# diver-j/melgan-multi

Measured on NVIDIA H100. Metric: generator_fwd_audio_frames_per_sec, higher is better.
Workload: dtype f32 in/out; products as 3 split-bf16 wgmma passes with fp32 accumulation (fp32-equivalent, ~1e-5)

## Files before the change

melgan_multi_b200/csrc/mg_common.cuh:

```cuda
#pragma once
#include <cuda_runtime.h>
#include <stdarg.h>
#include <stdint.h>
#include <stdio.h>

#include "../../include/melgan_b200.h"
#include "mg_layout.h"

namespace mg {

constexpr int kNumSMs = 132;

char *error_buffer();
int set_error(int code, const char *fmt, ...);

#define MG_CUDA_TRY(expr)                                                                     \
    do {                                                                                      \
        cudaError_t err__ = (expr);                                                           \
        if (err__ != cudaSuccess)                                                             \
            return ::mg::set_error(MG_ERR_CUDA, "%s failed: %s (%s:%d)", #expr,               \
                                   cudaGetErrorString(err__), __FILE__, __LINE__);            \
    } while (0)

__device__ __forceinline__ float lrelu(float x) { return fmaxf(x, x * kSlope); }

__device__ __forceinline__ void cp_async16(void *smem_dst, const void *gmem_src) {
    uint32_t d = (uint32_t)__cvta_generic_to_shared(smem_dst);
    asm volatile("cp.async.cg.shared.global [%0], [%1], 16;\n" ::"r"(d), "l"(gmem_src));
}
__device__ __forceinline__ void cp_async_commit() { asm volatile("cp.async.commit_group;\n" ::); }
template <int N>
__device__ __forceinline__ void cp_async_wait() {
    asm volatile("cp.async.wait_group %0;\n" ::"n"(N));
}

bool pdl_enabled();
template <class... KArgs, class... Args>
inline cudaError_t launch_ex(void (*kernel)(KArgs...), dim3 grid, dim3 block, size_t smem, cudaStream_t s, bool pdl, Args... args) {
    cudaLaunchConfig_t cfg{};
    cfg.gridDim = grid;
    cfg.blockDim = block;
    cfg.dynamicSmemBytes = smem;
    cfg.stream = s;
    cudaLaunchAttribute attr[1];
    int n = 0;
    if (pdl && pdl_enabled()) {
        attr[n].id = cudaLaunchAttributeProgrammaticStreamSerialization;
        attr[n].val.programmaticStreamSerializationAllowed = 1;
        ++n;
    }
    cfg.attrs = attr;
    cfg.numAttrs = n;
    return cudaLaunchKernelEx(&cfg, kernel, static_cast<KArgs>(args)...);
}

int launch_pack(const float *const *v, const float *const *g, const float *const *bias, float *packed,
                cudaStream_t s);
int launch_generator_simt(const float *packed, const float *mel, float *audio, int B, int T, float *ws,
                          cudaStream_t s, cudaEvent_t *ev = nullptr);
int generator_simt_num_launches();
int generator_tc_num_launches();
int generator_tc_fused_up();
int generator_tc_tail();
void generator_tc_set_tail(int mask);
const char *generator_tc_kernel_name(int i);
const char *generator_tc_kernel_config(int i, int T);
const char *resblock_config_name(int stage, int L);
int generator_tc_slices(int B, int T);
int launch_generator_tc(const float *packed, const float *mel, float *audio, int B, int T, float *ws, int *status,
                        cudaStream_t s, cudaEvent_t *ev = nullptr, const float *mel_host = nullptr, float *audio_host = nullptr);
int launch_gen_pre_tc(const float *mel, float *y, const float *packed, int B, int T, int *status, cudaStream_t s);
int launch_disc_post1_tc(const float *x, float *y, const uint8_t *wtc, const float *bias, int Bt, int L, int *status,
                         cudaStream_t s);
int launch_disc_post1_dgrad_tc(const float *dz, float *dx, const uint8_t *wtcT, const float *zero_bias, int Bt, int L, int *status,
                               cudaStream_t s);
int launch_disc_post1_wgrad_tc(const float *x, const float *dz, float *dw, float *db, int Bt, int L, int *status, cudaStream_t s);
size_t disc_scale_backward_workspace_bytes(int Bt, int L0);
int launch_disc_scale_backward(const void *blob, const float *x0, const float *const *fmap, const float *const *gfmap, float *gx0,
                               float *const *dw, float *const *db, int *reached, void *workspace, size_t workspace_bytes, int Bt,
                               int L0, int *status, cudaStream_t st);
size_t edge_bwd_workspace_bytes(int l, int Bt, int L);
// ... 34 lines not shown
```

melgan_multi_b200/csrc/mg_conv_tc.cu:

```cuda
#include "mg_common.cuh"
#include "mg_tc.cuh"

namespace mg {
using namespace tc;

template <int CIN_, int COUT_, int NTAP_, int KCA_, bool LRELU_OUT_, int N_>
struct ConvCfg {
    static constexpr int CIN = CIN_, COUT = COUT_, NTAP = NTAP_, PAD = NTAP_ / 2, KCA = KCA_;
    static constexpr bool LRELU_OUT = LRELU_OUT_;
    static constexpr int N = N_;
    static constexpr int NCG = COUT / N;
    static constexpr int ROWS = 128;
    static constexpr int AROWS = ROWS + 2 * PAD + 2;
    static constexpr int APITCH = AROWS * 16;
    static constexpr int ASLOT = 2 * (KCA / 8) * APITCH;
    static constexpr int BSLOT = 2 * 2 * N * 16;
    static constexpr int NSA = (CIN == KCA) ? 1 : 2, NSB = (N_ == 128) ? 8 : 4;
    static constexpr int NCONV = 128, NMW = 2;
    static constexpr int NT = NCONV + 128 * NMW + 32;
    static constexpr int SMEM_BYTES = NSA * ASLOT + NSB * BSLOT + (2 * NSA + 2 * NSB) * 8;
    static_assert(CIN % KCA == 0 && KCA % 16 == 0 && COUT % N == 0, "shape");
    static_assert(SMEM_BYTES + 1024 <= 227 * 1024, "shared memory budget");
};

// ... 135 lines not shown
        for (int ca = 0; ca < NCH; ca += 2) {
#pragma unroll
            for (int half = 0; half < 2; ++half) {
                const int cc = ca + half;
                if (cc < NCH) {
                    float *cur = half ? fb : fa, *nxt = half ? fa : fb;
                    if (cc + 1 < NCH) {
#pragma unroll
                        for (int j = 0; j < KCA; ++j) nxt[j] = inr0 ? __ldg(xrow + (size_t)((cc + 1) * KCA + j) * L) : 0.f;
                    }
                    if (ok && !mbar_wait(&emptyA[sa], pha ^ 1)) { ok = false; if (lane == 0) atomicExch(status, 24); }
                    uint8_t *slot = aring + sa * ASLOT;
                    store_row(slot, tid, cur);
                    tail_rows(slot, cc);
                    fence_proxy_async();
                    mbar_arrive(&fullA[sa]);
                    if (++sa == NSA) { sa = 0; pha ^= 1; }
                }
            }
        }
    }
}

template <class Cfg>
static int launch_conv_rows(const float *x, float *y, const uint8_t *wtc, const float *bias, int B, int L, int *status,
                            cudaStream_t s) {
    static bool configured = false;
    if (!configured) {
        MG_CUDA_TRY(cudaFuncSetAttribute(conv_rows_tc_kernel<Cfg>, cudaFuncAttributeMaxDynamicSharedMemorySize, Cfg::SMEM_BYTES));
        configured = true;
    }
    const long long vrows = (long long)B * (L + Cfg::PAD);
    const unsigned tiles = (unsigned)((vrows + Cfg::ROWS - 1) / Cfg::ROWS);
    MG_CUDA_TRY(launch_ex(conv_rows_tc_kernel<Cfg>, dim3(tiles, Cfg::NCG), dim3(Cfg::NT), Cfg::SMEM_BYTES, s, true, x, y, wtc, bias,
                          L, B, status));
    return MG_OK;
}

using PreCfg = ConvCfg<80, 512, 7, 80, false, kPreNG>;
using Post1Cfg = ConvCfg<1024, 1024, 5, 32, true, kPost1NG>;
using Post1DgradCfg = ConvCfg<1024, 1024, 5, 32, false, kPost1NG>;

int launch_gen_pre_tc(const float *mel, float *y, const float *packed, int B, int T, int *status, cudaStream_t s) {
    const uint8_t *wtc = reinterpret_cast<const uint8_t *>(packed) + tc_region_start() + tc_pre_offset();
    return launch_conv_rows<PreCfg>(mel, y, wtc, packed + bias_offset(0), B, T, status, s);
}

int launch_disc_post1_tc(const float *x, float *y, const uint8_t *wtc, const float *bias, int Bt, int L, int *status,
                         cudaStream_t s) {
    return launch_conv_rows<Post1Cfg>(x, y, wtc, bias, Bt, L, status, s);
}

int launch_disc_post1_dgrad_tc(const float *dz, float *dx, const uint8_t *wtcT, const float *zero_bias, int Bt, int L, int *status,
                               cudaStream_t s) {
    return launch_conv_rows<Post1DgradCfg>(dz, dx, wtcT, zero_bias, Bt, L, status, s);
}

}
```

melgan_multi_b200/csrc/mg_res_tc.cu:

```cuda
#include <stdlib.h>
#include <string.h>

#include "mg_common.cuh"
#include "mg_tc.cuh"

namespace mg {
using namespace tc;

template <int C_, int NRB_, int RPW_, int NCP_, int NSTAGE_, bool POST_ = false, bool UPF_ = false, int UPT_ = 0>
struct RbCfg {
    static constexpr int C = C_, NRB = NRB_, RPW = RPW_, NCP = NCP_, NSTAGE = NSTAGE_, UPT = UPT_;
    static constexpr bool POST = POST_;
    static constexpr bool UPF = UPF_;
    static constexpr int P = 64 * NRB;
    static constexpr int NWG = NRB / RPW * NCP;
    static constexpr int NCONS = 128 * NWG;
    static constexpr int NT = NCONS + 32;
    static constexpr int NCW = C / NCP;
    static constexpr int SLACK = 16;
    static constexpr int HALO = 16 + (POST ? 3 : 0);
    static constexpr int HL = HALO + (UPT_ ? 1 : 0);
    static constexpr int PVALID = P - HALO - HL;
    static constexpr int ROWS = P + 2 * SLACK;
    static constexpr int XPITCH = ROWS * 16;
    static constexpr int KP = C / 8;
    static constexpr int XBYTES = KP * XPITCH;
    static constexpr int KC = tc_kc(C);
    static constexpr int CHUNK = tc_chunk_bytes(C);
    static constexpr int HALF = CHUNK / 2;
    static constexpr int NCHUNK = tc_chunks_per_conv(C);
    static constexpr int KSL = C / KC;
    static constexpr int TNG = UPT == 8 ? 32 : C / 2, TN = (UPT ? UPT : 1) * TNG, TNCG = (C / 2) / TNG;
    static constexpr int TSLOT = UPT == 8 ? 16384 : 128 * UPT * TNG, TNSLOT = UPT ? TNCG * (C / 16) * (UPT == 8 ? 2 : 1) : 0;
    static_assert(UPT == 0 || ((UPT == 2 || UPT == 8) && TN == C && TSLOT <= CHUNK && !POST_ && !UPF_), "tail ConvT shape");
    static_assert(UPT != 8 || NCW == 128, "stride-8 tail: each column part stores four phases of a channel as one float4");
    static constexpr int UROWS = P / 2 + 2, UPITCH = UROWS * 16, NPB = NRB / 2, UKSL = 2 * C / KC, NUPCH = UPF ? 4 * UKSL : 0;
    static constexpr int SPITCH = P + 4;
    static_assert(!UPF || (NCP == 1 && NPB <= NWG && 2 * KP * UPITCH <= XBYTES && C * SPITCH * 4 <= 2 * XBYTES),
                  "fused ConvT must fit the X region");
    static_assert(!POST || (C == 32 && NCP == 1), "conv_post fusion is for the 32-channel stage");
    static constexpr int SMEM_BYTES = 2 * XBYTES + NSTAGE * CHUNK + 2 * C * 4 + 2 * NSTAGE * 8;
    static_assert(SMEM_BYTES + 1024 <= 227 * 1024, "shared memory budget");
    static_assert(XPITCH / 16 < 16384, "LBO field");
    static_assert(NRB % RPW == 0 && C % NCP == 0 && NCW % 32 == 0, "warpgroup split");
};

template <int RPW, int R>
__device__ __forceinline__ void acc_fence2(float (&a)[RPW][R]) {
#pragma unroll
    for (int r = 0; r < RPW; ++r) acc_fence<R>(a[r]);
}

template <class Cfg>
__global__ void __launch_bounds__(Cfg::NT, 1)
resblock_tc_kernel(const float *__restrict__ x, float *__restrict__ y, const float *__restrict__ packed, int stage, int L, int nB,
                   int *__restrict__ status, long long *__restrict__ trace) {
    constexpr int C = Cfg::C, P = Cfg::P, SLACK = Cfg::SLACK, HALO = Cfg::HALO, HL = Cfg::HL, PVS = Cfg::PVALID;
    constexpr int XPITCH = Cfg::XPITCH, XBYTES = Cfg::XBYTES, KC = Cfg::KC, CHUNK = Cfg::CHUNK, NSTAGE = Cfg::NSTAGE;
    constexpr int NCONS = Cfg::NCONS, NCP = Cfg::NCP, NCW = Cfg::NCW, RPW = Cfg::RPW, KSL = Cfg::KSL, NA = NCW / 2;
    extern __shared__ __align__(1024) uint8_t smem[];
    uint8_t *Xh = smem, *Xl = smem + XBYTES, *ring = smem + 2 * XBYTES;
    float *pend = reinterpret_cast<float *>(ring + NSTAGE * CHUNK);
    float *b1s = pend + C;
    uint64_t *full = reinterpret_cast<uint64_t *>(b1s + C);
    uint64_t *empty = full + NSTAGE;

    const int tid = threadIdx.x, warp = tid >> 5, lane = tid & 31;
    const int b = blockIdx.y, stile = blockIdx.x;
    const int o = stile == 0 ? 0 : (P - HALO) + (stile - 1) * PVS - HL;
    const int p_lo = stile == 0 ? 0 : HL, p_hi = (o + P >= L) ? P : P - HALO;
    const bool interior = (o >= 0 && o + P <= L);
    const int l0 = 5 + 6 * stage;
    const uint8_t *tc_base = reinterpret_cast<const uint8_t *>(packed) + tc_region_start();

    if (tid == 0) {
        for (int s = 0; s < NSTAGE; ++s) {
            mbar_init(&full[s], 1);
            mbar_init(&empty[s], Cfg::NWG);
        }
        fence_mbar_init();
    }
    for (int i = Cfg::UPF ? 1 << 30 : tid; i < 2 * Cfg::KP * 2 * SLACK; i += Cfg::NT) {
        const int r = i % (2 * SLACK), kp = (i / (2 * SLACK)) % Cfg::KP, hl = i / (2 * SLACK * Cfg::KP);
        const int row = r < SLACK ? r : P + r;
        *reinterpret_cast<uint4 *>((hl ? Xl : Xh) + kp * XPITCH + row * 16) = make_uint4(0, 0, 0, 0);
    }
    for (int i = tid; i < C; i += Cfg::NT) pend[i] = 0.f;
    fence_proxy_async();
    __syncthreads();
    const bool tr = trace && blockIdx.y == 0 && blockIdx.x == (gridDim.x > 1 ? 1u : 0u) && tid == 0;
#define MG_TR(slot) do { if (tr) trace[slot] = clock64(); } while (0)

    if (warp == NCONS / 32) {
        if (lane == 0) {
            int s = 0, ph = 0;
            bool ok = true;
            auto put = [&](const uint8_t *src, uint32_t bytes) {
                if (!ok || !mbar_wait(&empty[s], ph ^ 1)) { ok = false; return; }
                mbar_arrive_expect_tx(&full[s], bytes);
                bulk_g2s(ring + s * CHUNK, src, bytes, &full[s]);
                if (++s == NSTAGE) { s = 0; ph ^= 1; }
            };
            if constexpr (Cfg::UPF) {
                const uint8_t *src = tc_base + tc_upf_offset(stage);
                for (int i = 0; i < Cfg::NUPCH; ++i) put(src + (size_t)i * CHUNK, CHUNK);
            }
            for (int conv = 0; conv < 6; ++conv) {
                const uint8_t *src = tc_base + tc_res_offset(l0 + (conv >> 1) + 3 * (conv & 1));
                for (int i = 0; i < Cfg::NCHUNK; ++i) put(src + (size_t)i * CHUNK, CHUNK);
            }
            if constexpr (Cfg::UPT != 0) {
                const uint8_t *src = tc_base + tc_up_offset(stage + 1);
                for (int i = 0; i < Cfg::TNSLOT; ++i) put(src + (size_t)i * Cfg::TSLOT, Cfg::TSLOT);
            }
            if (!ok) atomicExch(status, 2);
        }
        return;
    }

    const int wgi = warp >> 2, t = tid & 127, q = lane & 3;
    const int rb0 = (wgi / NCP) * RPW, c0 = (wgi % NCP) * NCW;
    const uint64_t adesc_t = desc_template(XPITCH, 128), bdesc_t = desc_template(C * 16, 128);
    const uint32_t xh_addr = smem_u32(Xh), xl_addr = smem_u32(Xl), ring_addr = smem_u32(ring);
    float R[RPW][NA], D[RPW][NA];
    int s = 0, ph = 0, ps = -1;
    bool ok = true;
    auto chunk_begin = [&]() -> uint32_t {
        ok &= mbar_wait(&full[s], ph);
        acc_fence2(R);
        acc_fence2(D);
        wgmma_fence();
        return ring_addr + s * CHUNK;
    };
    auto chunk_end = [&]() {
        wgmma_commit();
        wgmma_wait<1>();
        if (t == 0 && ps >= 0) mbar_arrive(&empty[ps]);
        ps = s;
        if (++s == NSTAGE) { s = 0; ph ^= 1; }
    };
    auto drain = [&]() {
        wgmma_wait<0>();
        acc_fence2(R);
        acc_fence2(D);
        if (t == 0 && ps >= 0) mbar_arrive(&empty[ps]);
        ps = -1;
    };
    auto sync_cons = [&]() { named_bar_sync(1, NCONS); };
    auto write_x = [&](float (&A)[RPW][NA], const float *bsrc, bool keep_last) {
#pragma unroll
        for (int r = 0; r < RPW; ++r)
#pragma unroll
            for (int h = 0; h < 2; ++h) {
                const int p = (rb0 + r) * 64 + frag_row(t, h), tp = o + p;
                const bool inr = interior || (tp >= 0 && tp < L);
                uint8_t *xh = Xh + (c0 >> 3) * XPITCH + (p + SLACK) * 16 + q * 4, *xl = xh + XBYTES;
#pragma unroll
                for (int k = 0; k < NCW / 8; ++k) {
                    const int col = c0 + 8 * k + 2 * q;
                    const float2 bb = *reinterpret_cast<const float2 *>(bsrc + col);
                    const float f0 = inr ? lrelu(A[r][4 * k + 2 * h] + bb.x) : 0.f;
                    const float f1 = inr ? lrelu(A[r][4 * k + 2 * h + 1] + bb.y) : 0.f;
                    uint32_t hi, lo;
                    split2_bf16(f0, f1, hi, lo);
                    *reinterpret_cast<uint32_t *>(xh + k * XPITCH) = hi;
                    *reinterpret_cast<uint32_t *>(xl + k * XPITCH) = lo;
                    if (keep_last && tp == L - 1) *reinterpret_cast<float2 *>(b1s + col) = make_float2(f0, f1);
                }
            }
    };
    auto conv_mma = [&](float (&A)[RPW][NA], int dil, bool fresh, int conv) {
        MG_TR(64 + 3 * conv);
#pragma unroll 1
        for (int ch = 0; ch < Cfg::NCHUNK; ++ch) {
            const int tap = ch / KSL, ks = ch % KSL;
            const uint64_t bbase = desc_at(bdesc_t, chunk_begin() + c0 * 16);
            if (ch == 0) MG_TR(65 + 3 * conv);
            const uint32_t arow = (SLACK + rb0 * 64 + (tap - 1) * dil) * 16 + ks * (KC / 8) * XPITCH;
#pragma unroll
            for (int pass = 0; pass < 3; ++pass)
#pragma unroll
                for (int k16 = 0; k16 < KC / 16; ++k16) {
                    const uint64_t bdesc = bbase + (uint64_t)(((pass == 2 ? Cfg::HALF : 0) + 2 * k16 * (C * 16)) >> 4);
                    const uint64_t adesc = desc_at(adesc_t, (pass == 1 ? xl_addr : xh_addr) + arow + 2 * k16 * XPITCH);
#pragma unroll
                    for (int r = 0; r < RPW; ++r)
                        wgmma_bf16<NCW>(A[r], adesc + (uint64_t)(r * 64), bdesc, !(fresh && ch == 0 && pass == 0 && k16 == 0));
                }
            chunk_end();
        }
        MG_TR(66 + 3 * conv);
        drain();
    };

    pdl_wait();
    MG_TR(0);
    if constexpr (Cfg::UPF) {
        constexpr int UROWS = Cfg::UROWS, UPITCH = Cfg::UPITCH, SPITCH = Cfg::SPITCH, UKSL = Cfg::UKSL;
        const int Lin = L >> 1, s0 = (o >> 1) - 1;
#pragma unroll 1
        for (int idx = tid; idx < UROWS * 2 * Cfg::KP; idx += NCONS) {
            const int i = idx % UROWS, kp = idx / UROWS, sp = s0 + i;
            const bool inr = (sp >= 0 && sp < Lin);
            const float *xp = x + ((size_t)b * 2 * C + 8 * kp) * Lin + (inr ? sp : 0);
// ... 49 lines not shown
                    }
                }
            }
        }
        sync_cons();
#pragma unroll
        for (int r = 0; r < RPW; ++r)
#pragma unroll
            for (int j = 0; j < NA; ++j) {
                const int p = (rb0 + r) * 64 + frag_row(t, (j >> 1) & 1);
                R[r][j] = stg[(size_t)frag_col(q, (j & ~3) | (j & 1)) * SPITCH + p];
            }
        sync_cons();
        for (int i = tid; i < 2 * Cfg::KP * 2 * SLACK; i += NCONS) {
            const int r = i % (2 * SLACK), kp = (i / (2 * SLACK)) % Cfg::KP, hl = i / (2 * SLACK * Cfg::KP);
            const int row = r < SLACK ? r : P + r;
            *reinterpret_cast<uint4 *>((hl ? Xl : Xh) + kp * XPITCH + row * 16) = make_uint4(0, 0, 0, 0);
        }
    } else {
#pragma unroll
        for (int r = 0; r < RPW; ++r)
#pragma unroll
            for (int h = 0; h < 2; ++h) {
                const int p = (rb0 + r) * 64 + frag_row(t, h), tp = o + p;
                const bool inr = (tp >= 0 && tp < L);
                const float *xp = x + (size_t)b * C * L + (inr ? tp : 0);
#pragma unroll
                for (int k = 0; k < NCW / 8; ++k)
#pragma unroll
                    for (int e = 0; e < 2; ++e)
                        R[r][4 * k + 2 * h + e] = inr ? __ldg(xp + (size_t)(c0 + frag_col(q, 4 * k + e)) * L) : 0.f;
            }
    }
    write_x(R, pend, false);
    fence_proxy_async();
    sync_cons();
    MG_TR(1);

#pragma unroll 1
    for (int pr = 0; pr < 3; ++pr) {
        const float *bias1 = packed + bias_offset(l0 + pr);
        for (int c = tid; c < C; c += NCONS) b1s[c] = __ldg(bias1 + c);
        MG_TR(2 + 6 * pr);
        conv_mma(D, pr == 0 ? 1 : pr == 1 ? 3 : 9, true, 2 * pr);
        MG_TR(3 + 6 * pr);
        sync_cons();
        write_x(D, b1s, false);
        fence_proxy_async();
        sync_cons();
        MG_TR(4 + 6 * pr);
        const float *bias2 = packed + bias_offset(l0 + 3 + pr);
        for (int c = tid; c < C; c += NCONS) pend[c] += __ldg(bias2 + c);
        MG_TR(5 + 6 * pr);
        conv_mma(R, 1, false, 2 * pr + 1);
        MG_TR(6 + 6 * pr);
        sync_cons();
        if (pr < 2 || Cfg::UPT != 0) {
            write_x(R, pend, Cfg::UPT != 0 && pr == 2);
            fence_proxy_async();
            sync_cons();
        }
        MG_TR(7 + 6 * pr);
    }

    if constexpr (Cfg::POST) {
        pdl_trigger();
        float *Q = reinterpret_cast<float *>(Xh);
        float *wpost = reinterpret_cast<float *>(Xl);
        for (int i = tid; i < 32 * 8; i += NCONS)
            wpost[i] = (i & 7) < kPostK ? __ldg(packed + weight_offset(29) + (i >> 3) * kPostK + (i & 7)) : 0.f;
        sync_cons();
#pragma unroll
        for (int r = 0; r < RPW; ++r)
#pragma unroll
            for (int h = 0; h < 2; ++h) {
                const int p = (rb0 + r) * 64 + frag_row(t, h), tp = o + p;
                const bool inr = (tp >= 0 && tp < L);
                float qk[kPostK];
#pragma unroll
                for (int k = 0; k < kPostK; ++k) qk[k] = 0.f;
#pragma unroll
                for (int k = 0; k < NCW / 8; ++k)
#pragma unroll
                    for (int e = 0; e < 2; ++e) {
                        const int ci = frag_col(q, 4 * k + e);
                        const float a = inr ? lrelu(R[r][4 * k + 2 * h + e] + pend[ci]) : 0.f;
                        const float4 w0 = *reinterpret_cast<const float4 *>(wpost + ci * 8);
                        const float4 w1 = *reinterpret_cast<const float4 *>(wpost + ci * 8 + 4);
                        qk[0] = fmaf(w0.x, a, qk[0]); qk[1] = fmaf(w0.y, a, qk[1]); qk[2] = fmaf(w0.z, a, qk[2]);
                        qk[3] = fmaf(w0.w, a, qk[3]); qk[4] = fmaf(w1.x, a, qk[4]); qk[5] = fmaf(w1.y, a, qk[5]);
                        qk[6] = fmaf(w1.z, a, qk[6]);
                    }
#pragma unroll
                for (int k = 0; k < kPostK; ++k) {
// ... 99 lines not shown
                            }
                    } else {
                        float *yb = y + (size_t)b * COT * Lout + (own ? 2 * sg - PADT : 0);
#pragma unroll
                        for (int k = 0; k < NCW / 8; ++k)
#pragma unroll
                            for (int e = 0; e < 2; ++e) {
                                const int col = c0 + frag_col(q, 4 * k + e), phi = col / TNG, co = col % TNG;
                                if (phi == 0 ? lo_ok : hi_ok) yb[(size_t)co * Lout + phi] = D[r][4 * k + 2 * h + e] + __ldg(tbias + co);
                            }
                    }
                }
        }
    } else {
        pdl_trigger();
#pragma unroll
        for (int r = 0; r < RPW; ++r)
#pragma unroll
            for (int h = 0; h < 2; ++h) {
                const int p = (rb0 + r) * 64 + frag_row(t, h), tp = o + p;
                if (p >= p_lo && p < p_hi && tp < L) {
                    float *yp = y + (size_t)b * C * L + tp;
#pragma unroll
                    for (int k = 0; k < NCW / 8; ++k)
#pragma unroll
                        for (int e = 0; e < 2; ++e) {
                            const int col = c0 + frag_col(q, 4 * k + e);
                            yp[(size_t)col * L] = R[r][4 * k + 2 * h + e] + pend[col];
                        }
                }
            }
    }
    if (!ok && t == 0) atomicExch(status, 3);
    MG_TR(20);
#undef MG_TR
}

template <class Cfg>
static int launch_resblock(const float *x, float *y, const float *packed, int stage, int B, int L, int *status,
                           long long *trace, cudaStream_t s) {
    static bool configured = false;
    if (!configured) {
        MG_CUDA_TRY(cudaFuncSetAttribute(resblock_tc_kernel<Cfg>, cudaFuncAttributeMaxDynamicSharedMemorySize, Cfg::SMEM_BYTES));
        configured = true;
    }
    constexpr int P = Cfg::P, PVS = Cfg::PVALID;
    const int ntiles = 1 + (L > P ? (L - P + PVS - 1) / PVS : 0);
    if (B > 65535) return set_error(MG_ERR_INVALID_ARGUMENT, "launch_resblock_tc: batch %d exceeds the grid", B);
    MG_CUDA_TRY(launch_ex(resblock_tc_kernel<Cfg>, dim3(ntiles, B), dim3(Cfg::NT), Cfg::SMEM_BYTES, s, true, x, y, packed, stage,
                          L, B, status, trace));
    return MG_OK;
}

template <class Cfg>
static const char *cfg_name() {
    static char buf[96];
    snprintf(buf, sizeof(buf), "resblock_tc_kernel<RbCfg<%d,%d,%d,%d,%d,%d,%d,%d>>", Cfg::C, Cfg::NRB, Cfg::RPW, Cfg::NCP, Cfg::NSTAGE,
             (int)Cfg::POST, (int)Cfg::UPF, Cfg::UPT);
    return buf;
}

using Rb0 = RbCfg<256, 1, 1, 2, 4>;
using Rb1 = RbCfg<128, 2, 1, 1, 4>;
using Rb2 = RbCfg<64, 4, 1, 1, 3>;
using Rb3 = RbCfg<32, 8, 2, 1, 4>;
using Rb3Post = RbCfg<32, 8, 2, 1, 4, true>;
using Up2Rb2 = RbCfg<64, 4, 1, 1, 3, false, true>;
using Up3Rb3 = RbCfg<32, 8, 2, 1, 4, false, true>;
using Up3Rb3Post = RbCfg<32, 8, 2, 1, 4, true, true>;
using Rb0Up1 = RbCfg<256, 1, 1, 2, 4, false, false, 8>;
using Rb1Up2 = RbCfg<128, 2, 1, 1, 4, false, false, 2>;
using Rb2Up3 = RbCfg<64, 4, 1, 1, 3, false, false, 2>;

int launch_resblock_tc(const float *x, float *y, const float *packed, int stage, int B, int L, int *status, cudaStream_t s,
                       long long *trace) {
    switch (stage) {
        case 0: return launch_resblock<Rb0>(x, y, packed, 0, B, L, status, trace, s);
        case 1: return launch_resblock<Rb1>(x, y, packed, 1, B, L, status, trace, s);
        case 2: return launch_resblock<Rb2>(x, y, packed, 2, B, L, status, trace, s);
        case 3: return launch_resblock<Rb3>(x, y, packed, 3, B, L, status, trace, s);
        case 4: return launch_resblock<Rb3Post>(x, y, packed, 3, B, L, status, trace, s);
        case 12: return launch_resblock<Up2Rb2>(x, y, packed, 2, B, L, status, trace, s);
        case 13: return launch_resblock<Up3Rb3>(x, y, packed, 3, B, L, status, trace, s);
        case 14: return launch_resblock<Up3Rb3Post>(x, y, packed, 3, B, L, status, trace, s);
        case 20: return launch_resblock<Rb0Up1>(x, y, packed, 0, B, L, status, trace, s);
        case 21: return launch_resblock<Rb1Up2>(x, y, packed, 1, B, L, status, trace, s);
        case 22: return launch_resblock<Rb2Up3>(x, y, packed, 2, B, L, status, trace, s);
    }
    return set_error(MG_ERR_INVALID_ARGUMENT, "launch_resblock_tc: stage %d", stage);
}

const char *resblock_config_name(int stage, int L) {
    (void)L;
    switch (stage) {
        case 0: return cfg_name<Rb0>();
        case 1: return cfg_name<Rb1>();
// ... 15 lines not shown
```

melgan_multi_b200/csrc/mg_tc.cuh:

```cuda
#pragma once
#include <cuda_bf16.h>
#include <stdint.h>

namespace mg {
namespace tc {

__device__ __forceinline__ uint32_t smem_u32(const void *p) { return (uint32_t)__cvta_generic_to_shared(p); }

__device__ __forceinline__ void mbar_init(uint64_t *bar, uint32_t count) {
    asm volatile("mbarrier.init.shared::cta.b64 [%0], %1;" ::"r"(smem_u32(bar)), "r"(count));
}
__device__ __forceinline__ void fence_mbar_init() { asm volatile("fence.mbarrier_init.release.cluster;" ::: "memory"); }
__device__ __forceinline__ void mbar_arrive_expect_tx(uint64_t *bar, uint32_t bytes) {
    asm volatile("mbarrier.arrive.expect_tx.shared::cta.b64 _, [%0], %1;" ::"r"(smem_u32(bar)), "r"(bytes) : "memory");
}
__device__ __forceinline__ void mbar_arrive(uint64_t *bar) {
    asm volatile("mbarrier.arrive.shared::cta.b64 _, [%0];" ::"r"(smem_u32(bar)) : "memory");
}
__device__ __forceinline__ bool mbar_try_wait(uint64_t *bar, uint32_t parity) {
    uint32_t ok;
    asm volatile(
        "{\n\t.reg .pred p;\n\t"
        "mbarrier.try_wait.parity.shared::cta.b64 p, [%1], %2;\n\t"
        "selp.b32 %0, 1, 0, p;\n\t}"
        : "=r"(ok)
        : "r"(smem_u32(bar)), "r"(parity)
        : "memory");
    return ok != 0;
}
__device__ __forceinline__ bool mbar_wait(uint64_t *bar, uint32_t parity, uint32_t max_spins = 1u << 24) {
    for (uint32_t i = 0; i < max_spins; ++i)
        if (mbar_try_wait(bar, parity)) return true;
    return false;
}

__device__ __forceinline__ void bulk_g2s(void *smem_dst, const void *gmem_src, uint32_t bytes, uint64_t *bar) {
    asm volatile("cp.async.bulk.shared::cluster.global.mbarrier::complete_tx::bytes [%0], [%1], %2, [%3];" ::"r"(
                     smem_u32(smem_dst)),
                 "l"(gmem_src), "r"(bytes), "r"(smem_u32(bar))
                 : "memory");
}
__device__ __forceinline__ void fence_proxy_async() { asm volatile("fence.proxy.async.shared::cta;" ::: "memory"); }

__device__ __forceinline__ void named_bar_sync(int id, int count) {
    asm volatile("bar.sync %0, %1;" ::"r"(id), "r"(count) : "memory");
}

__device__ __forceinline__ void pdl_trigger() { asm volatile("griddepcontrol.launch_dependents;" ::: "memory"); }
__device__ __forceinline__ void pdl_wait() { asm volatile("griddepcontrol.wait;" ::: "memory"); }

__device__ __forceinline__ uint64_t desc_template(uint32_t lbo_bytes, uint32_t sbo_bytes) {
    return ((uint64_t)((lbo_bytes >> 4) & 0x3FFF) << 16) | ((uint64_t)((sbo_bytes >> 4) & 0x3FFF) << 32);
}
__device__ __forceinline__ uint64_t desc_at(uint64_t tmpl, uint32_t saddr) { return tmpl | (uint64_t)((saddr >> 4) & 0x3FFF); }

__device__ __forceinline__ void wgmma_fence() { asm volatile("wgmma.fence.sync.aligned;" ::: "memory"); }
__device__ __forceinline__ void wgmma_commit() { asm volatile("wgmma.commit_group.sync.aligned;" ::: "memory"); }
template <int N>
__device__ __forceinline__ void wgmma_wait() {
    asm volatile("wgmma.wait_group.sync.aligned %0;" ::"n"(N) : "memory");
}
template <int R>
__device__ __forceinline__ void acc_fence(float *d) {
#pragma unroll
    for (int i = 0; i < R; ++i) asm volatile("" : "+f"(d[i])::"memory");
}
__device__ __forceinline__ int frag_row(int t, int h) { return 16 * (t >> 5) + ((t & 31) >> 2) + 8 * h; }
__host__ __device__ constexpr int frag_col(int lane_q, int j) { return 8 * (j >> 2) + 2 * lane_q + (j & 1); }

template <int N>
__device__ __forceinline__ void wgmma_bf16(float *d, uint64_t adesc, uint64_t bdesc, uint32_t scale_d);
#define MG_D8(i) "+f"(d[i]), "+f"(d[i + 1]), "+f"(d[i + 2]), "+f"(d[i + 3]), "+f"(d[i + 4]), "+f"(d[i + 5]), "+f"(d[i + 6]), "+f"(d[i + 7])
// ... 47 lines not shown
```

melgan_multi_b200/csrc/mg_up_tc.cu:

```cuda
#include "mg_common.cuh"
#include "mg_tc.cuh"

namespace mg {
using namespace tc;

template <int STAGE_>
struct UpCfg {
    static constexpr int STAGE = STAGE_;
    static constexpr int CIN = stage_cin(STAGE), COUT = stage_cout(STAGE), S = stage_stride(STAGE), PAD = stage_pad(STAGE);
    static constexpr int NG = up_ng(STAGE);
    static constexpr int NCG = COUT / NG;
    static constexpr int N = S * NG;
    static constexpr int NMW = (N > 128) ? 1 : 2;
    static constexpr int KCA = (S == 8) ? 64 : 32;
    static constexpr int ROWS = 64 * NMW;
    static constexpr int AROWS = ROWS + 8;
    static constexpr int APITCH = AROWS * 16;
    static constexpr int ASLOT = 2 * (KCA / 8) * APITCH;
    static constexpr int BSLOT = up_slot_bytes(STAGE);
    static constexpr int NSA = (CIN == KCA) ? 1 : 2, NSB = (S == 8) ? 4 : (CIN >= 128 ? 2 : 3);
    static constexpr int NCHUNK = CIN / 16;
    static constexpr int NCONV = 128;
    static constexpr int NT = NCONV + 128 * NMW + 32;
    static constexpr int SMEM_BYTES = NSA * ASLOT + NSB * BSLOT + (2 * NSA + 2 * NSB) * 8;
// ... 138 lines not shown
            for (int i = tid; i <= ROWS; i += NCONV) {
                const int v = r0 - 1 + i;
                const int item = v >= 0 ? v / Lv : 0, s = v - item * Lv;
                const bool inr = (v >= 0 && item < B && s < Lin);
                const float *xp = x + ((size_t)(inr ? item : 0) * CIN + ca * KCA) * Lin + (inr ? s : 0);
                float f[KCA];
#pragma unroll
                for (int j = 0; j < KCA; ++j) f[j] = inr ? __ldg(xp + (size_t)j * Lin) : 0.f;
#pragma unroll
                for (int kp = 0; kp < KCA / 8; ++kp) {
                    uint32_t h[4], l[4];
#pragma unroll
                    for (int e = 0; e < 4; ++e) split2_bf16(lrelu(f[8 * kp + 2 * e]), lrelu(f[8 * kp + 2 * e + 1]), h[e], l[e]);
                    *reinterpret_cast<uint4 *>(slot + kp * APITCH + i * 16) = make_uint4(h[0], h[1], h[2], h[3]);
                    *reinterpret_cast<uint4 *>(slot + (KCA / 8 + kp) * APITCH + i * 16) = make_uint4(l[0], l[1], l[2], l[3]);
                }
            }
            fence_proxy_async();
            mbar_arrive(&fullA[sa]);
            if (++sa == NSA) { sa = 0; pha ^= 1; }
        }
    }
}

template <class Cfg>
static int launch_convt(const float *x, float *y, const float *packed, int B, int Lin, int *status, cudaStream_t s) {
    static bool configured = false;
    if (!configured) {
        MG_CUDA_TRY(cudaFuncSetAttribute(convt_tc_kernel<Cfg>, cudaFuncAttributeMaxDynamicSharedMemorySize, Cfg::SMEM_BYTES));
        configured = true;
    }
    const long long vrows = (long long)B * (Lin + 1);
    dim3 grid((unsigned)((vrows + Cfg::ROWS - 1) / Cfg::ROWS), Cfg::NCG);
    MG_CUDA_TRY(launch_ex(convt_tc_kernel<Cfg>, grid, dim3(Cfg::NT), Cfg::SMEM_BYTES, s, true, x, y, packed, Lin, B, status));
    return MG_OK;
}

template <class Cfg>
__global__ void __launch_bounds__(Cfg::NCONV + 128 + 32, 1)
convt_resident_tc_kernel(const float *__restrict__ x, float *__restrict__ y, const float *__restrict__ packed, int Lin, int B,
                         int *__restrict__ status) {
    constexpr int CIN = Cfg::CIN, NG = Cfg::NG, N = Cfg::N, NCG = Cfg::NCG;
    constexpr int ROWS = 64, APITCH = Cfg::APITCH, BSLOT = Cfg::BSLOT, NCHUNK = Cfg::NCHUNK;
    constexpr int KPT = CIN / 8;
    constexpr int AHALF = KPT * APITCH;
    constexpr int NSB = 4, NCONV = Cfg::NCONV;
    static_assert(Cfg::S == 8 && N == 256 && Cfg::NMW == 1 && 2 * AHALF + NSB * BSLOT + 256 <= 227 * 1024, "resident ConvT shape");
    extern __shared__ __align__(1024) uint8_t smem[];
    uint8_t *abuf = smem, *bring = smem + 2 * AHALF;
    uint64_t *fullA = reinterpret_cast<uint64_t *>(bring + NSB * BSLOT);
    uint64_t *fullB = fullA + CIN / 64, *emptyB = fullB + NSB;

    const int tid = threadIdx.x, warp = tid >> 5, lane = tid & 31;
    const int r0 = blockIdx.x * ROWS;
    const int Lv = Lin + 1;

    if (tid == 0) {
        for (int s = 0; s < CIN / 64; ++s) mbar_init(&fullA[s], NCONV);
        for (int s = 0; s < NSB; ++s) { mbar_init(&fullB[s], 1); mbar_init(&emptyB[s], 1); }
        fence_mbar_init();
    }
    __syncthreads();

    if (warp == NCONV / 32 + 4) {
        if (lane == 0) {
            const uint8_t *src = reinterpret_cast<const uint8_t *>(packed) + tc_region_start() + tc_up_offset(Cfg::STAGE);
            int s = 0, ph = 0;
// ... 52 lines not shown
            for (int i = tid; i <= ROWS; i += NCONV) {
                const int v = r0 - 1 + i;
                const int item = v >= 0 ? v / Lv : 0, s = v - item * Lv;
                const bool inr = (v >= 0 && item < B && s < Lin);
                const float *xp = x + ((size_t)(inr ? item : 0) * CIN + ca * 64) * Lin + (inr ? s : 0);
                float f[64];
#pragma unroll
                for (int j = 0; j < 64; ++j) f[j] = inr ? __ldg(xp + (size_t)j * Lin) : 0.f;
#pragma unroll
                for (int kp = 0; kp < 8; ++kp) {
                    uint32_t h[4], l[4];
#pragma unroll
                    for (int e = 0; e < 4; ++e) split2_bf16(lrelu(f[8 * kp + 2 * e]), lrelu(f[8 * kp + 2 * e + 1]), h[e], l[e]);
                    *reinterpret_cast<uint4 *>(abuf + (ca * 8 + kp) * APITCH + i * 16) = make_uint4(h[0], h[1], h[2], h[3]);
                    *reinterpret_cast<uint4 *>(abuf + AHALF + (ca * 8 + kp) * APITCH + i * 16) = make_uint4(l[0], l[1], l[2], l[3]);
                }
            }
            fence_proxy_async();
            mbar_arrive(&fullA[ca]);
        }
    }
}

template <class Cfg>
static int launch_convt_resident(const float *x, float *y, const float *packed, int B, int Lin, int *status, cudaStream_t s) {
    constexpr int smem = 2 * (Cfg::CIN / 8) * Cfg::APITCH + 4 * Cfg::BSLOT + (Cfg::CIN / 64 + 2 * 4) * 8;
    static bool configured = false;
    if (!configured) {
        MG_CUDA_TRY(cudaFuncSetAttribute(convt_resident_tc_kernel<Cfg>, cudaFuncAttributeMaxDynamicSharedMemorySize, smem));
        configured = true;
    }
    const long long vrows = (long long)B * (Lin + 1);
    MG_CUDA_TRY(launch_ex(convt_resident_tc_kernel<Cfg>, dim3((unsigned)((vrows + 63) / 64)), dim3(Cfg::NCONV + 128 + 32), smem, s,
                          true, x, y, packed, Lin, B, status));
    return MG_OK;
}

int launch_convt_tc(const float *x, float *y, const float *packed, int stage, int B, int Lin, int *status, cudaStream_t s) {
    switch (stage) {
        case 0: return launch_convt<UpCfg<0>>(x, y, packed, B, Lin, status, s);
        case 1: return launch_convt_resident<UpCfg<1>>(x, y, packed, B, Lin, status, s);
        case 2: return launch_convt<UpCfg<2>>(x, y, packed, B, Lin, status, s);
        case 3: return launch_convt<UpCfg<3>>(x, y, packed, B, Lin, status, s);
    }
    return set_error(MG_ERR_INVALID_ARGUMENT, "launch_convt_tc: stage %d", stage);
}

}
```

melgan_multi_b200/csrc/mg_wgrad_tc.cu:

```cuda
#include "mg_common.cuh"
#include "mg_tc.cuh"

namespace mg {
using namespace tc;

namespace wg {
constexpr int C = 1024, NTAP = 5, PAD = 2;
constexpr int MT = 64, NTILE = 64;
constexpr int NPANEL = 4;
constexpr int NB = NTAP * NTILE;
constexpr int NMW = 2, NW = NB / NMW;
constexpr int APANEL = MT * 16 + 32, BPANEL = NB * 16 + 32;
constexpr int AHALF = NPANEL * APANEL, BHALF = NPANEL * BPANEL;
constexpr int ASTAGE = 2 * AHALF, BSTAGE = 2 * BHALF, STAGE = ASTAGE + BSTAGE;
constexpr int NSTAGE = 3;
constexpr int NCONV = 256;
constexpr int NT = NCONV + 128 * NMW;
constexpr int SMEM_BYTES = NSTAGE * STAGE + 2 * NSTAGE * 8 + 2 * NCONV * 4;
static_assert(SMEM_BYTES + 1024 <= 227 * 1024, "shared memory budget");
}

__device__ __forceinline__ void load4(const float *__restrict__ row, int p0, int L, bool vec, bool live, float *f) {
    if (vec) {
        float4 v = make_float4(0.f, 0.f, 0.f, 0.f);
// ... 109 lines not shown
            }
            fence_proxy_async();
            __syncwarp();
            if (lane == 0) mbar_arrive(&full[s]);
            if (++s == NSTAGE) { s = 0; ph ^= 1; }
        };
        float fa0[2][4], fb0[2][12], fa1[2][4], fb1[2][12];
        load_stage(0, fa0, fb0);
#pragma unroll 1
        for (int st = 0; st < nstages; st += 2) {
            if (st + 1 < nstages) load_stage(st + 1, fa1, fb1);
            store_stage(fa0, fb0);
            if (st + 1 < nstages) {
                if (st + 2 < nstages) load_stage(st + 2, fa0, fb0);
                store_stage(fa1, fb1);
            }
        }
#pragma unroll
        for (int u = 0; u < 2; ++u) dbsum[u * NCONV + tid] = acc_db[u];
    }
    __syncthreads();
    if (blockIdx.y == 0 && tid < MT) {
        const float *p = dbsum + (tid >> 5) * NCONV + (tid & 31) * 8;
        db[co0 + tid] = ((p[0] + p[1]) + (p[2] + p[3])) + ((p[4] + p[5]) + (p[6] + p[7]));
    }
}

int launch_disc_post1_wgrad_tc(const float *x, const float *dz, float *dw, float *db, int Bt, int L, int *status, cudaStream_t s) {
    static bool configured = false;
    if (!configured) {
        MG_CUDA_TRY(cudaFuncSetAttribute(post1_wgrad_tc_kernel, cudaFuncAttributeMaxDynamicSharedMemorySize, wg::SMEM_BYTES));
        configured = true;
    }
    MG_CUDA_TRY(launch_ex(post1_wgrad_tc_kernel, dim3(wg::C / wg::MT, wg::C / wg::NTILE), dim3(wg::NT), wg::SMEM_BYTES, s, false, x, dz,
                          dw, db, Bt, L, status));
    return MG_OK;
}

}
```

Before: 267.2 million.

## Run early ResBlock stages as thread-block clusters with DSMEM halo exchange and weight multicast

The ResBlock kernels for the 256- and 128-channel stages now launch as 4-CTA and 2-CTA clusters. Adjacent CTAs in a cluster swap boundary rows of the intermediate activations through distributed shared memory after each conv, rather than each tile recomputing a wide halo. The weight chunks are loaded once with TMA multicast to every CTA in the cluster, which cuts L2 traffic. In exchange there are extra cross-CTA mbarrier handshakes and cluster syncs, the empty barrier needs arrivals from every CTA, and cluster scheduling may reduce how many CTAs are resident.

```diff
diff --git a/melgan_multi_b200/csrc/mg_common.cuh b/melgan_multi_b200/csrc/mg_common.cuh
--- a/melgan_multi_b200/csrc/mg_common.cuh
+++ b/melgan_multi_b200/csrc/mg_common.cuh
@@ -36,17 +36,25 @@
 
 bool pdl_enabled();
 template <class... KArgs, class... Args>
-inline cudaError_t launch_ex(void (*kernel)(KArgs...), dim3 grid, dim3 block, size_t smem, cudaStream_t s, bool pdl, Args... args) {
+inline cudaError_t launch_ex(void (*kernel)(KArgs...), dim3 grid, dim3 block, size_t smem, cudaStream_t s, bool pdl, int cluster,
+                             Args... args) {
     cudaLaunchConfig_t cfg{};
     cfg.gridDim = grid;
     cfg.blockDim = block;
     cfg.dynamicSmemBytes = smem;
     cfg.stream = s;
-    cudaLaunchAttribute attr[1];
+    cudaLaunchAttribute attr[2];
     int n = 0;
     if (pdl && pdl_enabled()) {
         attr[n].id = cudaLaunchAttributeProgrammaticStreamSerialization;
         attr[n].val.programmaticStreamSerializationAllowed = 1;
+        ++n;
+    }
+    if (cluster > 1) {
+        attr[n].id = cudaLaunchAttributeClusterDimension;
+        attr[n].val.clusterDim.x = cluster;
+        attr[n].val.clusterDim.y = 1;
+        attr[n].val.clusterDim.z = 1;
         ++n;
     }
     cfg.attrs = attr;
diff --git a/melgan_multi_b200/csrc/mg_conv_tc.cu b/melgan_multi_b200/csrc/mg_conv_tc.cu
--- a/melgan_multi_b200/csrc/mg_conv_tc.cu
+++ b/melgan_multi_b200/csrc/mg_conv_tc.cu
@@ -191,7 +191,7 @@
     }
     const long long vrows = (long long)B * (L + Cfg::PAD);
     const unsigned tiles = (unsigned)((vrows + Cfg::ROWS - 1) / Cfg::ROWS);
-    MG_CUDA_TRY(launch_ex(conv_rows_tc_kernel<Cfg>, dim3(tiles, Cfg::NCG), dim3(Cfg::NT), Cfg::SMEM_BYTES, s, true, x, y, wtc, bias,
+    MG_CUDA_TRY(launch_ex(conv_rows_tc_kernel<Cfg>, dim3(tiles, Cfg::NCG), dim3(Cfg::NT), Cfg::SMEM_BYTES, s, true, 1, x, y, wtc, bias,
                           L, B, status));
     return MG_OK;
 }
diff --git a/melgan_multi_b200/csrc/mg_res_tc.cu b/melgan_multi_b200/csrc/mg_res_tc.cu
--- a/melgan_multi_b200/csrc/mg_res_tc.cu
+++ b/melgan_multi_b200/csrc/mg_res_tc.cu
@@ -7,9 +7,9 @@
 namespace mg {
 using namespace tc;
 
-template <int C_, int NRB_, int RPW_, int NCP_, int NSTAGE_, bool POST_ = false, bool UPF_ = false, int UPT_ = 0>
+template <int C_, int NRB_, int RPW_, int NCP_, int NSTAGE_, bool POST_ = false, bool UPF_ = false, int UPT_ = 0, int CS_ = 1>
 struct RbCfg {
-    static constexpr int C = C_, NRB = NRB_, RPW = RPW_, NCP = NCP_, NSTAGE = NSTAGE_, UPT = UPT_;
+    static constexpr int C = C_, NRB = NRB_, RPW = RPW_, NCP = NCP_, NSTAGE = NSTAGE_, UPT = UPT_, CS = CS_;
     static constexpr bool POST = POST_;
     static constexpr bool UPF = UPF_;
     static constexpr int P = 64 * NRB;
@@ -20,7 +20,6 @@
     static constexpr int SLACK = 16;
     static constexpr int HALO = 16 + (POST ? 3 : 0);
     static constexpr int HL = HALO + (UPT_ ? 1 : 0);
-    static constexpr int PVALID = P - HALO - HL;
     static constexpr int ROWS = P + 2 * SLACK;
     static constexpr int XPITCH = ROWS * 16;
     static constexpr int KP = C / 8;
@@ -39,7 +38,10 @@
     static_assert(!UPF || (NCP == 1 && NPB <= NWG && 2 * KP * UPITCH <= XBYTES && C * SPITCH * 4 <= 2 * XBYTES),
                   "fused ConvT must fit the X region");
     static_assert(!POST || (C == 32 && NCP == 1), "conv_post fusion is for the 32-channel stage");
-    static constexpr int SMEM_BYTES = 2 * XBYTES + NSTAGE * CHUNK + 2 * C * 4 + 2 * NSTAGE * 8;
+    static constexpr int PVB = CS * P - HALO - HL, XCH = 9;
+    static_assert(CS == 1 || ((CS == 2 || CS == 4) && !POST_ && !UPF_ && UPT_ == 0 && XCH <= SLACK && 2 * XCH <= P),
+                  "clusters are for the plain ResBlock");
+    static constexpr int SMEM_BYTES = 2 * XBYTES + NSTAGE * CHUNK + 2 * C * 4 + (2 * NSTAGE + (CS > 1 ? 2 : 0)) * 8;
     static_assert(SMEM_BYTES + 1024 <= 227 * 1024, "shared memory budget");
     static_assert(XPITCH / 16 < 16384, "LBO field");
     static_assert(NRB % RPW == 0 && C % NCP == 0 && NCW % 32 == 0, "warpgroup split");
@@ -55,20 +57,23 @@
 __global__ void __launch_bounds__(Cfg::NT, 1)
 resblock_tc_kernel(const float *__restrict__ x, float *__restrict__ y, const float *__restrict__ packed, int stage, int L, int nB,
                    int *__restrict__ status, long long *__restrict__ trace) {
-    constexpr int C = Cfg::C, P = Cfg::P, SLACK = Cfg::SLACK, HALO = Cfg::HALO, HL = Cfg::HL, PVS = Cfg::PVALID;
+    constexpr int C = Cfg::C, P = Cfg::P, SLACK = Cfg::SLACK, HALO = Cfg::HALO, HL = Cfg::HL;
     constexpr int XPITCH = Cfg::XPITCH, XBYTES = Cfg::XBYTES, KC = Cfg::KC, CHUNK = Cfg::CHUNK, NSTAGE = Cfg::NSTAGE;
     constexpr int NCONS = Cfg::NCONS, NCP = Cfg::NCP, NCW = Cfg::NCW, RPW = Cfg::RPW, KSL = Cfg::KSL, NA = NCW / 2;
+    constexpr int CS = Cfg::CS, XCH = Cfg::XCH;
     extern __shared__ __align__(1024) uint8_t smem[];
     uint8_t *Xh = smem, *Xl = smem + XBYTES, *ring = smem + 2 * XBYTES;
     float *pend = reinterpret_cast<float *>(ring + NSTAGE * CHUNK);
     float *b1s = pend + C;
     uint64_t *full = reinterpret_cast<uint64_t *>(b1s + C);
     uint64_t *empty = full + NSTAGE;
+    uint64_t *hfull = empty + NSTAGE, *hfree = hfull + 1;
 
     const int tid = threadIdx.x, warp = tid >> 5, lane = tid & 31;
-    const int b = blockIdx.y, stile = blockIdx.x;
-    const int o = stile == 0 ? 0 : (P - HALO) + (stile - 1) * PVS - HL;
-    const int p_lo = stile == 0 ? 0 : HL, p_hi = (o + P >= L) ? P : P - HALO;
+    const int b = blockIdx.y, clus = blockIdx.x / CS, crank = blockIdx.x % CS;
+    const int oc = clus == 0 ? 0 : (CS * P - HALO) + (clus - 1) * Cfg::PVB - HL;
+    const int o = oc + crank * P;
+    const int p_lo = (clus == 0 || crank > 0) ? 0 : HL, p_hi = (crank < CS - 1 || oc + CS * P >= L) ? P : P - HALO;
     const bool interior = (o >= 0 && o + P <= L);
     const int l0 = 5 + 6 * stage;
     const uint8_t *tc_base = reinterpret_cast<const uint8_t *>(packed) + tc_region_start();
@@ -76,7 +81,11 @@
     if (tid == 0) {
         for (int s = 0; s < NSTAGE; ++s) {
             mbar_init(&full[s], 1);
-            mbar_init(&empty[s], Cfg::NWG);
+            mbar_init(&empty[s], Cfg::NWG * CS);
+        }
+        if constexpr (CS > 1) {
+            mbar_init(hfull, 1);
+            mbar_init(hfree, (crank > 0) + (crank < CS - 1));
         }
         fence_mbar_init();
     }
@@ -88,17 +97,20 @@
     for (int i = tid; i < C; i += Cfg::NT) pend[i] = 0.f;
     fence_proxy_async();
     __syncthreads();
+    if constexpr (CS > 1) cluster_sync();
     const bool tr = trace && blockIdx.y == 0 && blockIdx.x == (gridDim.x > 1 ? 1u : 0u) && tid == 0;
 #define MG_TR(slot) do { if (tr) trace[slot] = clock64(); } while (0)
 
     if (warp == NCONS / 32) {
         if (lane == 0) {
-            int s = 0, ph = 0;
+            int s = 0, ph = 0, j = 0;
             bool ok = true;
             auto put = [&](const uint8_t *src, uint32_t bytes) {
                 if (!ok || !mbar_wait(&empty[s], ph ^ 1)) { ok = false; return; }
                 mbar_arrive_expect_tx(&full[s], bytes);
-                bulk_g2s(ring + s * CHUNK, src, bytes, &full[s]);
+                if constexpr (CS == 1) bulk_g2s(ring + s * CHUNK, src, bytes, &full[s]);
+                else if (j % CS == crank) bulk_g2s_multicast(ring + s * CHUNK, src, bytes, &full[s], (1 << CS) - 1);
+                ++j;
                 if (++s == NSTAGE) { s = 0; ph ^= 1; }
             };
             if constexpr (Cfg::UPF) {
@@ -115,6 +127,7 @@
             }
             if (!ok) atomicExch(status, 2);
         }
+        if constexpr (CS > 1) cluster_sync();
         return;
     }
 
@@ -125,6 +138,13 @@
     float R[RPW][NA], D[RPW][NA];
     int s = 0, ph = 0, ps = -1;
     bool ok = true;
+    auto release = [&](int slot) {
+        if constexpr (CS == 1) {
+            if (t == 0) mbar_arrive(&empty[slot]);
+        } else if (t < CS) {
+            mbar_arrive_remote(&empty[slot], t);
+        }
+    };
     auto chunk_begin = [&]() -> uint32_t {
         ok &= mbar_wait(&full[s], ph);
         acc_fence2(R);
@@ -135,7 +155,7 @@
     auto chunk_end = [&]() {
         wgmma_commit();
         wgmma_wait<1>();
-        if (t == 0 && ps >= 0) mbar_arrive(&empty[ps]);
+        if (ps >= 0) release(ps);
         ps = s;
         if (++s == NSTAGE) { s = 0; ph ^= 1; }
     };
@@ -143,10 +163,17 @@
         wgmma_wait<0>();
         acc_fence2(R);
         acc_fence2(D);
-        if (t == 0 && ps >= 0) mbar_arrive(&empty[ps]);
+        if (ps >= 0) release(ps);
         ps = -1;
     };
     auto sync_cons = [&]() { named_bar_sync(1, NCONS); };
+    const int nbr = tid == 0 ? crank - 1 : crank + 1;
+    const bool tells = tid < 2 && nbr >= 0 && nbr < CS;
+    auto x_read = [&]() {
+        sync_cons();
+        if constexpr (CS > 1)
+            if (tells) mbar_arrive_remote(hfree, nbr);
+    };
     auto write_x = [&](float (&A)[RPW][NA], const float *bsrc, bool keep_last) {
 #pragma unroll
         for (int r = 0; r < RPW; ++r)
@@ -169,7 +196,48 @@
                 }
             }
     };
+    bool border = false;
+#pragma unroll
+    for (int r = 0; r < RPW; ++r)
+#pragma unroll
+        for (int h = 0; h < 2; ++h) {
+            const int p = (rb0 + r) * 64 + frag_row(t, h);
+            border |= (crank > 0 && p < XCH) || (crank < CS - 1 && p >= P - XCH);
+        }
+    constexpr int NXC = 2 * Cfg::KP;
+    constexpr uint32_t XCB = XCH * 16;
+    constexpr int NW = NCONS / 32;
+    auto send_halo = [&]() {
+        for (int i = warp + NW * lane; i < 2 * NXC; i += NCONS) {
+            const int side = i / NXC, nb = side ? crank + 1 : crank - 1;
+            if (nb < 0 || nb >= CS) continue;
+            const uint32_t panel = xh_addr + (i % NXC) * XPITCH;
+            const int src = side ? P - XCH : 0, dst = side ? -XCH : P;
+            bulk_s2s_cluster(mapa(panel + (SLACK + dst) * 16, nb), panel + (SLACK + src) * 16, XCB, mapa(smem_u32(hfull), nb));
+        }
+    };
+    int hand = 0;
+    auto hand_off = [&](float (&A)[RPW][NA], const float *bsrc, bool keep_last) {
+        if constexpr (CS > 1) {
+            if (border && hand > 0) {
+                MG_TR(100 + 2 * hand);
+                ok &= mbar_wait(hfree, (hand - 1) & 1);
+                MG_TR(101 + 2 * hand);
+            }
+            if (tid == 0) mbar_arrive_expect_tx(hfull, ((crank > 0) + (crank < CS - 1)) * NXC * XCB);
+        }
+        write_x(A, bsrc, keep_last);
+        fence_proxy_async();
+        sync_cons();
+        if constexpr (CS > 1) send_halo();
+        ++hand;
+    };
     auto conv_mma = [&](float (&A)[RPW][NA], int dil, bool fresh, int conv) {
+        if constexpr (CS > 1) {
+            MG_TR(88 + 2 * conv);
+            ok &= mbar_wait(hfull, conv & 1);
+            MG_TR(89 + 2 * conv);
+        }
         MG_TR(64 + 3 * conv);
 #pragma unroll 1
         for (int ch = 0; ch < Cfg::NCHUNK; ++ch) {
@@ -285,9 +353,7 @@
                         R[r][4 * k + 2 * h + e] = inr ? __ldg(xp + (size_t)(c0 + frag_col(q, 4 * k + e)) * L) : 0.f;
             }
     }
-    write_x(R, pend, false);
-    fence_proxy_async();
-    sync_cons();
+    hand_off(R, pend, false);
     MG_TR(1);
 
 #pragma unroll 1
@@ -297,22 +363,16 @@
         MG_TR(2 + 6 * pr);
         conv_mma(D, pr == 0 ? 1 : pr == 1 ? 3 : 9, true, 2 * pr);
         MG_TR(3 + 6 * pr);
-        sync_cons();
-        write_x(D, b1s, false);
-        fence_proxy_async();
-        sync_cons();
+        x_read();
+        hand_off(D, b1s, false);
         MG_TR(4 + 6 * pr);
         const float *bias2 = packed + bias_offset(l0 + 3 + pr);
         for (int c = tid; c < C; c += NCONS) pend[c] += __ldg(bias2 + c);
         MG_TR(5 + 6 * pr);
         conv_mma(R, 1, false, 2 * pr + 1);
         MG_TR(6 + 6 * pr);
-        sync_cons();
-        if (pr < 2 || Cfg::UPT != 0) {
-            write_x(R, pend, Cfg::UPT != 0 && pr == 2);
-            fence_proxy_async();
-            sync_cons();
-        }
+        x_read();
+        if (pr < 2 || Cfg::UPT != 0) hand_off(R, pend, Cfg::UPT != 0 && pr == 2);
         MG_TR(7 + 6 * pr);
     }
 
@@ -478,6 +538,7 @@
             }
     }
     if (!ok && t == 0) atomicExch(status, 3);
+    if constexpr (CS > 1) cluster_sync();
     MG_TR(20);
 #undef MG_TR
 }
@@ -490,24 +551,40 @@
         MG_CUDA_TRY(cudaFuncSetAttribute(resblock_tc_kernel<Cfg>, cudaFuncAttributeMaxDynamicSharedMemorySize, Cfg::SMEM_BYTES));
         configured = true;
     }
-    constexpr int P = Cfg::P, PVS = Cfg::PVALID;
-    const int ntiles = 1 + (L > P ? (L - P + PVS - 1) / PVS : 0);
+    constexpr int CS = Cfg::CS, PC = CS * Cfg::P, PVB = Cfg::PVB;
+    const int nclusters = 1 + (L > PC ? (L - PC + PVB - 1) / PVB : 0);
     if (B > 65535) return set_error(MG_ERR_INVALID_ARGUMENT, "launch_resblock_tc: batch %d exceeds the grid", B);
-    MG_CUDA_TRY(launch_ex(resblock_tc_kernel<Cfg>, dim3(ntiles, B), dim3(Cfg::NT), Cfg::SMEM_BYTES, s, true, x, y, packed, stage,
-                          L, B, status, trace));
+    if (trace && CS > 1) {
+        cudaLaunchConfig_t cfg{};
+        cfg.gridDim = dim3(CS * nclusters, B);
+        cfg.blockDim = dim3(Cfg::NT);
+        cfg.dynamicSmemBytes = Cfg::SMEM_BYTES;
+        cudaLaunchAttribute attr;
+        attr.id = cudaLaunchAttributeClusterDimension;
+        attr.val.clusterDim.x = CS;
+        attr.val.clusterDim.y = attr.val.clusterDim.z = 1;
+        cfg.attrs = &attr;
+        cfg.numAttrs = 1;
+        int n = 0;
+        MG_CUDA_TRY(cudaOccupancyMaxActiveClusters(&n, resblock_tc_kernel<Cfg>, &cfg));
+        const long long v = n;
+        MG_CUDA_TRY(cudaMemcpy(trace + 127, &v, sizeof(v), cudaMemcpyHostToDevice));
+    }
+    MG_CUDA_TRY(launch_ex(resblock_tc_kernel<Cfg>, dim3(CS * nclusters, B), dim3(Cfg::NT), Cfg::SMEM_BYTES, s, true, CS, x, y, packed,
+                          stage, L, B, status, trace));
     return MG_OK;
 }
 
 template <class Cfg>
 static const char *cfg_name() {
     static char buf[96];
-    snprintf(buf, sizeof(buf), "resblock_tc_kernel<RbCfg<%d,%d,%d,%d,%d,%d,%d,%d>>", Cfg::C, Cfg::NRB, Cfg::RPW, Cfg::NCP, Cfg::NSTAGE,
-             (int)Cfg::POST, (int)Cfg::UPF, Cfg::UPT);
+    snprintf(buf, sizeof(buf), "resblock_tc_kernel<RbCfg<%d,%d,%d,%d,%d,%d,%d,%d,%d>>", Cfg::C, Cfg::NRB, Cfg::RPW, Cfg::NCP,
+             Cfg::NSTAGE, (int)Cfg::POST, (int)Cfg::UPF, Cfg::UPT, Cfg::CS);
     return buf;
 }
 
-using Rb0 = RbCfg<256, 1, 1, 2, 4>;
-using Rb1 = RbCfg<128, 2, 1, 1, 4>;
+using Rb0 = RbCfg<256, 1, 1, 2, 4, false, false, 0, 4>;
+using Rb1 = RbCfg<128, 2, 1, 1, 4, false, false, 0, 2>;
 using Rb2 = RbCfg<64, 4, 1, 1, 3>;
 using Rb3 = RbCfg<32, 8, 2, 1, 4>;
 using Rb3Post = RbCfg<32, 8, 2, 1, 4, true>;
diff --git a/melgan_multi_b200/csrc/mg_tc.cuh b/melgan_multi_b200/csrc/mg_tc.cuh
--- a/melgan_multi_b200/csrc/mg_tc.cuh
+++ b/melgan_multi_b200/csrc/mg_tc.cuh
@@ -34,10 +34,35 @@
     return false;
 }
 
+__device__ __forceinline__ uint32_t mapa(uint32_t addr, uint32_t rank) {
+    uint32_t r;
+    asm volatile("mapa.shared::cluster.u32 %0, %1, %2;" : "=r"(r) : "r"(addr), "r"(rank));
+    return r;
+}
+__device__ __forceinline__ void mbar_arrive_remote(uint64_t *bar, uint32_t rank) {
+    asm volatile("mbarrier.arrive.shared::cluster.b64 _, [%0];" ::"r"(mapa(smem_u32(bar), rank)) : "memory");
+}
+__device__ __forceinline__ void cluster_sync() {
+    asm volatile("barrier.cluster.arrive.release;\n\tbarrier.cluster.wait.acquire;" ::: "memory");
+}
+
 __device__ __forceinline__ void bulk_g2s(void *smem_dst, const void *gmem_src, uint32_t bytes, uint64_t *bar) {
     asm volatile("cp.async.bulk.shared::cluster.global.mbarrier::complete_tx::bytes [%0], [%1], %2, [%3];" ::"r"(
                      smem_u32(smem_dst)),
                  "l"(gmem_src), "r"(bytes), "r"(smem_u32(bar))
+                 : "memory");
+}
+__device__ __forceinline__ void bulk_g2s_multicast(void *smem_dst, const void *gmem_src, uint32_t bytes, uint64_t *bar,
+                                                   uint16_t cta_mask) {
+    asm volatile(
+        "cp.async.bulk.shared::cluster.global.mbarrier::complete_tx::bytes.multicast::cluster [%0], [%1], %2, [%3], %4;" ::"r"(
+            smem_u32(smem_dst)),
+        "l"(gmem_src), "r"(bytes), "r"(smem_u32(bar)), "h"(cta_mask)
+        : "memory");
+}
+__device__ __forceinline__ void bulk_s2s_cluster(uint32_t dst, uint32_t src, uint32_t bytes, uint32_t bar) {
+    asm volatile("cp.async.bulk.shared::cluster.shared::cta.mbarrier::complete_tx::bytes [%0], [%1], %2, [%3];" ::"r"(dst), "r"(src),
+                 "r"(bytes), "r"(bar)
                  : "memory");
 }
 __device__ __forceinline__ void fence_proxy_async() { asm volatile("fence.proxy.async.shared::cta;" ::: "memory"); }
diff --git a/melgan_multi_b200/csrc/mg_up_tc.cu b/melgan_multi_b200/csrc/mg_up_tc.cu
--- a/melgan_multi_b200/csrc/mg_up_tc.cu
+++ b/melgan_multi_b200/csrc/mg_up_tc.cu
@@ -194,7 +194,7 @@
     }
     const long long vrows = (long long)B * (Lin + 1);
     dim3 grid((unsigned)((vrows + Cfg::ROWS - 1) / Cfg::ROWS), Cfg::NCG);
-    MG_CUDA_TRY(launch_ex(convt_tc_kernel<Cfg>, grid, dim3(Cfg::NT), Cfg::SMEM_BYTES, s, true, x, y, packed, Lin, B, status));
+    MG_CUDA_TRY(launch_ex(convt_tc_kernel<Cfg>, grid, dim3(Cfg::NT), Cfg::SMEM_BYTES, s, true, 1, x, y, packed, Lin, B, status));
     return MG_OK;
 }
 
@@ -313,7 +313,7 @@
     }
     const long long vrows = (long long)B * (Lin + 1);
     MG_CUDA_TRY(launch_ex(convt_resident_tc_kernel<Cfg>, dim3((unsigned)((vrows + 63) / 64)), dim3(Cfg::NCONV + 128 + 32), smem, s,
-                          true, x, y, packed, Lin, B, status));
+                          true, 1, x, y, packed, Lin, B, status));
     return MG_OK;
 }
 
diff --git a/melgan_multi_b200/csrc/mg_wgrad_tc.cu b/melgan_multi_b200/csrc/mg_wgrad_tc.cu
--- a/melgan_multi_b200/csrc/mg_wgrad_tc.cu
+++ b/melgan_multi_b200/csrc/mg_wgrad_tc.cu
@@ -165,7 +165,7 @@
         MG_CUDA_TRY(cudaFuncSetAttribute(post1_wgrad_tc_kernel, cudaFuncAttributeMaxDynamicSharedMemorySize, wg::SMEM_BYTES));
         configured = true;
     }
-    MG_CUDA_TRY(launch_ex(post1_wgrad_tc_kernel, dim3(wg::C / wg::MT, wg::C / wg::NTILE), dim3(wg::NT), wg::SMEM_BYTES, s, false, x, dz,
+    MG_CUDA_TRY(launch_ex(post1_wgrad_tc_kernel, dim3(wg::C / wg::MT, wg::C / wg::NTILE), dim3(wg::NT), wg::SMEM_BYTES, s, false, 1, x, dz,
                           dw, db, Bt, L, status));
     return MG_OK;
 }
```

Result: faster. 279.5 million (median of 6 runs) (+4.6%).
